# westlake-repl/IDvs.MoRec

Hardware: AMD Instinct MI355X
Metric: user-sequences/sec end-to-end train step, SASRec+BERT-base (higher is better)
Workload: dtype fp16

## Files before the change

### idvs/morec_amd/_lib.py

```python
from __future__ import annotations

import ctypes as C
import os

import torch

_HERE = os.path.dirname(os.path.abspath(__file__))
LIB_PATH = os.environ.get("MOREC_HIP_LIB") or os.path.join(_HERE, "libmorec_hip.so")

F32, BF16, F16 = 0, 1, 2
ACT_NONE, ACT_GELU, ACT_RELU = 0, 1, 2
DACT_MUL = 3


class MorecError(RuntimeError):
    pass


class GemmDesc(C.Structure):
    _fields_ = [("M", C.c_int), ("N", C.c_int), ("K", C.c_int), ("lda", C.c_int), ("ldb", C.c_int), ("ldc", C.c_int),
                ("in_dtype", C.c_int), ("out_dtype", C.c_int), ("act", C.c_int), ("dact", C.c_int),
                ("accumulate", C.c_int), ("split_k", C.c_int), ("alpha", C.c_float), ("aux_deriv", C.c_int)]


# ... 24 lines not shown
                ("pad0", C.c_int32), ("drop_seed", C.c_uint64), ("drop_seed_mixed", C.c_uint64), ("reserved", C.c_int32 * 2)]


class SwinAttnDesc(C.Structure):
    _fields_ = [("n_img", C.c_int), ("H", C.c_int), ("W", C.c_int), ("window", C.c_int), ("shift", C.c_int),
                ("heads", C.c_int), ("dh", C.c_int), ("scale", C.c_float), ("dtype", C.c_int)]


_P = C.c_void_p
_SIGS = {
    "morec_strerror": (C.c_char_p, [C.c_int]),
    "morec_version": (C.c_int, []),
    "morec_tuning_set": (C.c_int, [C.c_char_p, C.c_int]),
    "morec_det_scratch_reserve": (C.c_int, [C.c_size_t, C.c_void_p]),
    "morec_stream_wait_stream": (C.c_int, [_P, _P]),
    "morec_gemm_nt": (C.c_int, [C.POINTER(GemmDesc), _P, _P, _P, _P, _P, _P, _P]),
    "morec_gemm_nt_colsum": (C.c_int, [C.POINTER(GemmDesc), _P, _P, _P, _P, _P, _P, _P, _P, _P]),
    "morec_gemm_colsum_workspace_bytes": (C.c_size_t, [C.c_int, C.c_int]),
    "morec_gemm_plan": (C.c_int, [C.POINTER(GemmDesc), C.c_int, C.c_int, C.c_int, C.c_int, C.c_int, C.POINTER(GemmPlanInfo)]),
    "morec_gemm_tn": (C.c_int, [_P, _P, _P, C.c_int, C.c_int, C.c_int, C.c_int, C.c_int, C.c_int, C.c_int, C.c_int, C.c_int, _P, _P]),
    "morec_gemm_tn_workspace_bytes": (C.c_size_t, [C.c_int, C.c_int, C.c_int]),
    "morec_mlp_dact_recompute_supported": (C.c_int, [C.c_int, C.c_int, C.c_int, C.c_int]),
    "morec_mlp_dact_recompute_workspace_bytes": (C.c_size_t, [C.c_int]),
    "morec_mlp_dact_recompute": (C.c_int, [_P, _P, _P, _P, _P, _P, _P, _P, C.c_int, C.c_int, C.c_int, C.c_int, _P]),
    "morec_transpose": (C.c_int, [_P, _P, C.c_int, C.c_int, C.c_int, C.c_int, C.c_int, C.c_int, _P]),
    "morec_transpose_batch": (C.c_int, [_P, C.c_int, C.c_int, C.c_int, _P]),
    "morec_cast": (C.c_int, [_P, _P, C.c_size_t, C.c_int, C.c_int, _P]),
    "morec_split_bf16x3": (C.c_int, [_P, _P, C.c_int, C.c_int, C.c_int, C.c_int, C.c_int, _P]),
    "morec_act_bwd": (C.c_int, [_P, _P, _P, C.c_size_t, C.c_int, C.c_int, _P]),
    "morec_scaled_sum": (C.c_int, [_P, _P, _P, _P, C.c_size_t, C.c_float, C.c_int, _P]),
# ... 90 lines not shown
```

### idvs/morec_amd/csrc/attention.hip

```cpp
#include <stdio.h>
#include <stdlib.h>
#include "common.hpp"

namespace {
template <int TB>
struct Tile {
    static constexpr int TP = 8 * TB;
    static constexpr int PP = TP + 4;
};

struct AttnArgs {
    const void* qkv;
    const float* key_keep;
    void* ctx;
    void* dqkv;
    int n_seq, T, n_heads, dh;
    int causal;
    float scale, mask_value;
    DropRng drop;
    const int32_t* cu;
    int total_rows;
};

template <typename T, int DC, int TB>
// ... 670 lines not shown
    if (rc != MOREC_E_UNSUPPORTED) return rc;
    warn_valu_fallback(d);
    (void)block;
    if (d->T > Tile<8>::TP) return launch_long<true>(d, a, grid, s);
    return launch_valu<true>(d, a, grid, s);
}

extern "C" int morec_attn_bwd_dbias(const morec_attn_desc* d, const void* qkv, const float* key_keep, const void* dctx,
                                    void* dqkv, int rows, float* dbias, float* ws, size_t ws_bytes, void* stream) {
    int rc = check_desc(d);
    if (rc) return rc;
    if (!qkv || !key_keep || !dctx || !dqkv || !dbias || rows <= 0) return MOREC_E_ARG;
    const int H3 = 3 * d->n_heads * d->dh;
    hipStream_t s = reinterpret_cast<hipStream_t>(stream);
    if (ws && ws_bytes >= (size_t)d->n_seq * H3 * sizeof(float)) {
        rc = morec_attn_mfma_launch(d, qkv, key_keep, const_cast<void*>(dctx), dqkv, true, s, ws);
        if (rc == MOREC_OK) return colsum_f32_launch(ws, dbias, d->n_seq, H3, s);
        if (rc != MOREC_E_UNSUPPORTED) return rc;
    }
    rc = morec_attn_bwd(d, qkv, key_keep, dctx, dqkv, stream);
    if (rc) return rc;
    return morec_colsum(dqkv, dbias, rows, H3, H3, d->dtype, stream);
}
```

### idvs/morec_amd/csrc/capi.hip

```cpp
#include <atomic>
#include <mutex>
#include <stdlib.h>
#include "common.hpp"

extern "C" const char* morec_strerror(int code) {
    switch (code) {
        case MOREC_OK: return "ok";
        case MOREC_E_ARG: return "MOREC_E_ARG: null pointer or non-positive size";
        case MOREC_E_ALIGN: return "MOREC_E_ALIGN: pointer/pitch not 16-byte aligned or size not a vector multiple";
        case MOREC_E_UNSUPPORTED: return "MOREC_E_UNSUPPORTED: shape outside kernel limits";
        case MOREC_E_DTYPE: return "MOREC_E_DTYPE: unsupported dtype combination";
        case MOREC_E_COMM: return "MOREC_E_COMM: an RCCL call failed (morec_comm_last_error)";
        default: break;
    }
    if (code > 0) return hipGetErrorString(static_cast<hipError_t>(code));
    return "unknown morec error";
}

extern "C" int morec_version(void) { return 105; }

static const uint64_t* g_drop_seed_src = nullptr;
const uint64_t* morec_drop_seed_src() { return g_drop_seed_src; }
extern "C" int morec_dropout_seed_source(const void* dev_u64) {
    if (reinterpret_cast<uintptr_t>(dev_u64) & 7u) return MOREC_E_ALIGN;
    g_drop_seed_src = reinterpret_cast<const uint64_t*>(dev_u64);
    return MOREC_OK;
}

static float* det_scratch_impl(hipStream_t s, size_t n, bool may_grow) {
    struct Slot { hipStream_t s; int dev; float* p; size_t n; unsigned long long used; };
    static Slot slots[16];
    static int n_slots = 0;
    static unsigned long long tick = 0;
    static std::mutex mu;
    std::lock_guard<std::mutex> lock(mu);
    int dev = 0;
    (void)hipGetDevice(&dev);
    hipStreamCaptureStatus cap = hipStreamCaptureStatusNone;
    if (hipStreamIsCapturing(s, &cap) != hipSuccess) { (void)hipGetLastError(); cap = hipStreamCaptureStatusNone; }
    const bool capturing = cap != hipStreamCaptureStatusNone;
    Slot* sl = nullptr;
    for (int i = 0; i < n_slots; ++i)
        if (slots[i].s == s && slots[i].dev == dev) sl = &slots[i];
    if (!sl) {
        if (capturing || !may_grow) return nullptr;
        if (n_slots < 16) {
            sl = &slots[n_slots++];
        } else {
            for (int i = 0; i < n_slots; ++i)
                if (slots[i].dev == dev && (!sl || slots[i].used < sl->used)) sl = &slots[i];
            if (!sl) return nullptr;
            (void)hipDeviceSynchronize();
            if (sl->p) (void)hipFree(sl->p);
        }
        *sl = Slot{s, dev, nullptr, 0, 0};
    }
    sl->used = ++tick;
    if (sl->n < n) {
        if (capturing || !may_grow) return nullptr;
        if (sl->p) {
            (void)hipStreamSynchronize(s);
            (void)hipFree(sl->p);
            sl->p = nullptr; sl->n = 0;
        }
        size_t want = n + n / 4;
        if (want < ((size_t)1 << 20)) want = (size_t)1 << 20;
        if (hipMalloc(reinterpret_cast<void**>(&sl->p), want * sizeof(float)) != hipSuccess) { (void)hipGetLastError(); sl->p = nullptr; return nullptr; }
        sl->n = want;
    }
    return sl->p;
}
float* morec_det_scratch(hipStream_t s, size_t n) { return det_scratch_impl(s, n, true); }
extern "C" int morec_det_scratch_reserve(size_t n_floats, void* stream) {
    return det_scratch_impl(reinterpret_cast<hipStream_t>(stream), n_floats, true) ? MOREC_OK : (int)hipErrorOutOfMemory;
}

__global__ __launch_bounds__(256) void det_fold_add_kernel(const float* __restrict__ part, float* __restrict__ dst, int n_parts, size_t n, size_t stride) {
    __shared__ float red[16][17];
    const int c = threadIdx.x & 15, g = threadIdx.x >> 4;
    const size_t j = blockIdx.x * (size_t)16 + c;
    float a0 = 0.f, a1 = 0.f, a2 = 0.f, a3 = 0.f;
    if (j < n) {
        int p = g;
        for (; p + 48 < n_parts; p += 64) {
            a0 += part[(size_t)p * stride + j];
            a1 += part[(size_t)(p + 16) * stride + j];
            a2 += part[(size_t)(p + 32) * stride + j];
            a3 += part[(size_t)(p + 48) * stride + j];
        }
        for (; p < n_parts; p += 16) a0 += part[(size_t)p * stride + j];
    }
    red[g][c] = (a0 + a1) + (a2 + a3);
    __syncthreads();
    if (g == 0 && j < n) {
        float t = 0.f;
#pragma unroll
        for (int k = 0; k < 16; ++k) t += red[k][c];
        dst[j] += t;
    }
}
int morec_det_fold_add(const float* part, float* dst, int n_parts, size_t n, size_t stride, hipStream_t s) {
    if (n == 0 || n_parts <= 0) return MOREC_OK;
    hipLaunchKernelGGL(det_fold_add_kernel, dim3((unsigned)((n + 15) / 16)), dim3(256), 0, s, part, dst, n_parts, n, stride);
    MOREC_CHECK_LAUNCH();
    return MOREC_OK;
}

extern "C" int morec_stream_wait_stream(void* waiting, void* signal) {
    static hipEvent_t ring[256];
    static std::atomic<unsigned> next{0};
    static const hipError_t made = [] {
        for (auto& e : ring) {
            const hipError_t rc = hipEventCreateWithFlags(&e, hipEventDisableTiming);
            if (rc != hipSuccess) return rc;
        }
        return hipSuccess;
    }();
    if (made != hipSuccess) return (int)made;
    hipEvent_t e = ring[next.fetch_add(1u, std::memory_order_relaxed) & 255u];
// ... 61 lines not shown
```

### idvs/morec_amd/csrc/common.hpp

```cpp
#pragma once
#include <hip/hip_runtime.h>
#include <stdint.h>
#include <math.h>
#include <type_traits>
#include "morec_hip.h"
#include "tuning.hpp"

#define MOREC_WAVE 64

struct bf16 {
    unsigned short v;
};

typedef __attribute__((ext_vector_type(8))) __bf16 bf16x8_t;
typedef __attribute__((ext_vector_type(4))) float f32x4_t;

__device__ __forceinline__ float bf2f(bf16 x) { return __uint_as_float(((uint32_t)x.v) << 16); }
__device__ __forceinline__ float bfbits2f(uint32_t lo16) { return __uint_as_float(lo16 << 16); }
typedef __attribute__((ext_vector_type(2))) float f32x2_t;
typedef __attribute__((ext_vector_type(2))) __bf16 bf16x2_t;
typedef __attribute__((ext_vector_type(4))) __bf16 bf16x4_t;
__device__ __forceinline__ unsigned short f2bf_bits(float f) { return __builtin_bit_cast(unsigned short, (__bf16)f); }
__device__ __forceinline__ uint32_t pack_bf16x2(float lo, float hi) {
    const f32x2_t v = {lo, hi};
// ... 336 lines not shown
        case MOREC_F16: f((f16*)nullptr); return true;
        default: return false;
    }
}
#define MOREC_TAG_T(tag) typename std::remove_pointer<decltype(tag)>::type
#define MOREC_CHECK_LAUNCH()                        \
    do {                                            \
        hipError_t e__ = hipGetLastError();         \
        if (e__ != hipSuccess) return (int)e__;     \
    } while (0)

bool morec_deterministic();
void morec_set_deterministic(int on);
float* morec_det_scratch(hipStream_t s, size_t n);
int morec_det_fold_add(const float* part, float* dst, int n_parts, size_t n, size_t stride, hipStream_t s);

__device__ __forceinline__ int xcd_remap(int bid, int nwg) {
    const int q = nwg >> 3, r = nwg & 7, xcd = bid & 7, idx = bid >> 3;
    const int base = (xcd < r) ? xcd * (q + 1) : r * (q + 1) + (xcd - r) * q;
    return base + idx;
}
```

### idvs/morec_amd/csrc/gemm.hip

```cpp
#include "gemm_nt_generic.hpp"


extern "C" int morec_gemm_nt(const morec_gemm_desc* d, const void* A, const void* B, void* C, const float* bias,
                             void* aux_out, const void* dact_in, void* stream) {
    return morec_gemm_nt_colsum(d, A, B, C, bias, aux_out, dact_in, nullptr, nullptr, stream);
}

extern "C" size_t morec_gemm_colsum_workspace_bytes(int M, int N) {
    return (size_t)((M + 31) / 32) * (size_t)N * sizeof(float);
}

static int check_gemm_desc(const morec_gemm_desc* d, bool aligned, bool dact_in, bool aux_out, bool colsum) {
    if (colsum) {
        if (d->dact == MOREC_ACT_NONE || d->accumulate != 0 || d->split_k > 1) return MOREC_E_UNSUPPORTED;
        const int os_ = elt_size(d->out_dtype);
        if ((d->N * os_) % 16 || (d->ldc * os_) % 16) return MOREC_E_UNSUPPORTED;
    }
    if (d->M <= 0 || d->N <= 0 || d->K <= 0) return MOREC_E_ARG;
    const int es = elt_size(d->in_dtype), os = elt_size(d->out_dtype);
    if (!aligned) return MOREC_E_ALIGN;
    if ((d->lda * es) % 16 || (d->ldb * es) % 16 || (d->K * es) % 16) return MOREC_E_ALIGN;
    if (d->N % 4 || (d->ldc * os) % (4 * os) || d->ldc % 4) return MOREC_E_ALIGN;
    if (d->split_k > 1 && d->accumulate != 2) return MOREC_E_ARG;
    if (d->accumulate == 2 && d->out_dtype != MOREC_F32) return MOREC_E_DTYPE;
// ... 8 lines not shown
    return (d->N * os) % 16 == 0 && (d->ldc * os) % 16 == 0;
}

extern "C" int morec_gemm_nt_colsum(const morec_gemm_desc* d, const void* A, const void* B, void* C, const float* bias,
                                    void* aux_out, const void* dact_in, float* colsum_out, float* workspace, void* stream) {
    if (!d || !A || !B || !C) return MOREC_E_ARG;
    if (colsum_out && !workspace) return MOREC_E_ARG;
    const bool aligned = aligned16(A) && aligned16(B) && aligned16(C) && (!bias || aligned16(bias));
    const int rc = check_gemm_desc(d, aligned, dact_in, aux_out, colsum_out);
    if (rc) return rc;
    GemmArgs a{};
    a.A = A; a.B = B; a.C = C; a.bias = bias; a.aux_out = aux_out; a.dact_in = dact_in;
    a.M = d->M; a.N = d->N; a.K = d->K; a.lda = d->lda; a.ldb = d->ldb; a.ldc = d->ldc;
    a.act = d->act; a.dact = d->dact; a.accumulate = d->accumulate; a.alpha = d->alpha;
    a.aux_deriv = d->aux_deriv;
    a.colsum = colsum_out ? workspace : nullptr;
    a.colsum_dst = colsum_out;
    a.vec_store = rows_16_byte_addressable(d) && (!aux_out || aligned16(aux_out));
    const GemmOperands o{bias != nullptr, aux_out != nullptr, dact_in != nullptr, colsum_out != nullptr, a.vec_store != 0, aligned16(bias)};
    const GemmPlan p = gemm_plan(*d, o, tuning(), gemm8p_cu_count());
    a.wave_epilogue = p.wave_epilogue;
    hipStream_t s = reinterpret_cast<hipStream_t>(stream);
    switch (p.family) {
        case GEMM_SKINNY: return gemm_skinny_launch(p, a, s);
        case GEMM_SKINNY_WIDE: return gemm_skinny_wide_launch(p, a, s);
        case GEMM_TWO_W: return gemm2w_launch(p, a, s);
        case GEMM_EIGHT_P: return gemm8p_launch(p, a, s);
        case GEMM_SMALL: return gemm_small_launch(p, a, s);
        case GEMM_GENERIC:
            if (p.in_dtype == MOREC_F16) return gemm_nt_f16_launch(p, a, s);
// ... 204 lines not shown
            float t = 0.f;
#pragma unroll
            for (int r = 0; r < 16; ++r) t += part[r][threadIdx.x];
            if (det) out[(size_t)blockIdx.y * N + c] = t;
            else atomicAdd(out + c, t);
        }
    }
}

int colsum_f32_launch(const float* in, float* out, int rows, int N, hipStream_t s) {
    const int cb = (N + 63) / 64;
    int rpb = (int)(((long)rows * cb / 512 + 15) & ~15L);
    rpb = rpb < 16 ? 16 : rpb > 512 ? 512 : rpb;
    if ((long)rows * N <= (1L << 20) && rows <= 512) rpb = 512;
    dim3 grid(cb, (rows + rpb - 1) / rpb);
    if (grid.y > 1 && morec_deterministic()) {
        float* part = morec_det_scratch(s, (size_t)grid.y * N);
        if (!part) return (int)hipErrorOutOfMemory;
        hipLaunchKernelGGL((colsum_kernel<float>), grid, dim3(256), 0, s, in, part, rows, N, N, rpb, 1);
        MOREC_CHECK_LAUNCH();
        return morec_det_fold_add(part, out, (int)grid.y, (size_t)N, (size_t)N, s);
    }
    hipLaunchKernelGGL((colsum_kernel<float>), grid, dim3(256), 0, s, in, out, rows, N, N, rpb);
    MOREC_CHECK_LAUNCH();
    return MOREC_OK;
}

extern "C" int morec_colsum(const void* in, float* out, int M, int N, int ld, int dtype, void* stream) {
    if (!in || !out || M <= 0 || N <= 0) return MOREC_E_ARG;
    if (N % 4 || ld % 4) return MOREC_E_ALIGN;
    const int rpb = 512;
    dim3 grid((N + 63) / 64, (M + rpb - 1) / rpb);
    hipStream_t s = reinterpret_cast<hipStream_t>(stream);
    float* part = nullptr;
    if (grid.y > 1 && morec_deterministic()) {
        part = morec_det_scratch(s, (size_t)grid.y * N);
        if (!part) return (int)hipErrorOutOfMemory;
    }
    if (!by_dtype(dtype, [&](auto* t) {
            using T = MOREC_TAG_T(t);
            hipLaunchKernelGGL((colsum_kernel<T>), grid, dim3(256), 0, s, (const T*)in, part ? part : out, M, N, ld, rpb, part ? 1 : 0);
        }))
        return MOREC_E_DTYPE;
    MOREC_CHECK_LAUNCH();
    if (part) return morec_det_fold_add(part, out, (int)grid.y, (size_t)N, (size_t)N, s);
    return MOREC_OK;
}

template <typename T>
__global__ void act_bwd_kernel(const T* __restrict__ dy, const T* __restrict__ pre, T* __restrict__ out, size_t n4,
// ... 66 lines not shown
```

### idvs/morec_amd/csrc/gemm_skinny_wide.hip

```cpp
#include "gemm_core.hpp"
#include "gemm_args.hpp"

namespace {
typedef __attribute__((ext_vector_type(4))) unsigned int u32x4_t;
constexpr int TR = 32;
constexpr int THREADS = 512;
constexpr int NW = 8;

struct WArgs {
    const bf16* A;
    const bf16* B;
    bf16* C;
    const float* bias;
    const bf16* A2;
    const bf16* B2;
    float* colsum_ws;
    int M, N, K, lda, ldb, ldc, lda2, ldb2, tiles;
};

template <int N>
__device__ __forceinline__ void vm_wait() {
    asm volatile("s_waitcnt vmcnt(%0)" ::"n"(N) : "memory");
}
__device__ __forceinline__ void bar_lds() {
// ... 251 lines not shown

extern "C" int morec_mlp_dact_recompute(const void* dY, const void* W2t, const void* X, const void* W1, const float* b1, void* dU,
                                        float* colsum_out, float* workspace, int M, int N, int K, int dtype, void* stream) {
    if (!dY || !W2t || !X || !W1 || !dU || M <= 0 || N <= 0 || K <= 0) return MOREC_E_ARG;
    if (colsum_out && !workspace) return MOREC_E_ARG;
    if (!is_h16(dtype)) return MOREC_E_DTYPE;
    if (!dual_class_exists(M, N, K, dtype)) return MOREC_E_UNSUPPORTED;
    if (b1 && (reinterpret_cast<uintptr_t>(b1) & 15u)) return MOREC_E_ALIGN;
    if (!aligned16(dY) || !aligned16(W2t) || !aligned16(X) || !aligned16(W1) || !aligned16(dU)) return MOREC_E_ALIGN;
    hipStream_t s = reinterpret_cast<hipStream_t>(stream);
    WArgs k{};
    k.A = reinterpret_cast<const bf16*>(dY); k.B = reinterpret_cast<const bf16*>(W2t); k.C = reinterpret_cast<bf16*>(dU);
    k.A2 = reinterpret_cast<const bf16*>(X); k.B2 = reinterpret_cast<const bf16*>(W1);
    k.bias = b1;
    k.M = M; k.N = N; k.K = K; k.lda = K; k.ldb = K; k.ldc = N; k.lda2 = K; k.ldb2 = K; k.tiles = (M + TR - 1) / TR;
    k.colsum_ws = colsum_out ? workspace : nullptr;
    return dtype == MOREC_F16 ? dispatch_wide<f16, 1, true>(k, colsum_out, s) : dispatch_wide<bf16, 1, true>(k, colsum_out, s);
}
```

### idvs/morec_amd/csrc/swin.hip

```cpp
#include <algorithm>
#include "common.hpp"

namespace {
constexpr int DH = 32;

struct SwinAttnArgs {
    const void* qkv;
    const float* bias_t;
    void* ctx;
    const void* dctx;
    void* dqkv;
    float* dbias_t;
    float* dbias_part;
    int n_img, H, W, shift, heads;
    float scale;
    int n_win_total, wpb;
};

template <int WS>
__device__ __forceinline__ void token_geom(const SwinAttnArgs& a, int img, int wr, int wc, int t, int& row, int& reg) {
    const int wy = t / WS, wx = t - wy * WS;
    const int ys = wr * WS + wy, xs = wc * WS + wx;
    int y = ys + a.shift, x = xs + a.shift;
    if (y >= a.H) y -= a.H;
// ... 468 lines not shown
    hipStream_t s = reinterpret_cast<hipStream_t>(stream);
    rc = morec_swin_attn_mfma_launch(d, qkv, bias_t, const_cast<void*>(ctx), dctx, dqkv, dbias_t, true, s);
    if (rc != MOREC_E_UNSUPPORTED) return rc;
    dim3 grid(gx, d->heads), block(64);
    const int NT2 = d->window * d->window * d->window * d->window;
    if (dbias_t && morec_deterministic()) {
        a.dbias_part = morec_det_scratch(s, (size_t)d->heads * gx * NT2);
        if (!a.dbias_part) return (int)hipErrorOutOfMemory;
    }
    if (d->dtype == MOREC_F32) hipLaunchKernelGGL((swin_attn_bwd_kernel<float, 7>), grid, block, 0, s, a);
    else if (d->dtype == MOREC_F16) hipLaunchKernelGGL((swin_attn_bwd_kernel<f16, 7>), grid, block, 0, s, a);
    else hipLaunchKernelGGL((swin_attn_bwd_kernel<bf16, 7>), grid, block, 0, s, a);
    MOREC_CHECK_LAUNCH();
    if (a.dbias_part)
        for (int h = 0; h < d->heads; ++h) {
            rc = morec_det_fold_add(a.dbias_part + (size_t)h * gx * NT2, dbias_t + (size_t)h * NT2, gx, (size_t)NT2, (size_t)NT2, s);
            if (rc) return rc;
        }
    return MOREC_OK;
}

extern "C" int morec_swin_bias_expand(const float* table, float* bias_t, int window, int heads, void* stream) {
    if (!table || !bias_t || window <= 0 || heads <= 0) return MOREC_E_ARG;
    const int n = heads * window * window * window * window;
    hipLaunchKernelGGL(swin_bias_expand_kernel, dim3((n + 255) / 256), dim3(256), 0, reinterpret_cast<hipStream_t>(stream),
                       table, bias_t, window, heads);
    MOREC_CHECK_LAUNCH();
    return MOREC_OK;
}

extern "C" int morec_swin_bias_reduce(const float* dbias_t, float* dtable, int window, int heads, void* stream) {
// ... 122 lines not shown
    MOREC_CHECK_LAUNCH();
    return MOREC_OK;
}

extern "C" int morec_swin_attn_bwd_dbias(const morec_swin_attn_desc* d, const void* qkv, const float* bias_t, const void* ctx,
                                         const void* dctx, void* dqkv, float* dbias_t, float* dbqkv, float* ws, size_t ws_bytes,
                                         void* stream) {
    int rc = check_attn(d);
    if (rc) return rc;
    if (!qkv || !bias_t || !ctx || !dctx || !dqkv || !dbqkv) return MOREC_E_ARG;
    const int C3 = 3 * d->heads * d->dh;
    const long rows = (long)d->n_img * d->H * d->W;
    hipStream_t s = reinterpret_cast<hipStream_t>(stream);
    if (ws) {
        int need = 0;
        rc = morec_swin_attn_mfma_launch(d, qkv, bias_t, const_cast<void*>(ctx), dctx, dqkv, dbias_t, true, s, ws,
                                         (long)(ws_bytes / (C3 * sizeof(float))), &need);
        if (rc == MOREC_OK) return colsum_f32_launch(ws, dbqkv, need, C3, s);
        if (rc != MOREC_E_UNSUPPORTED) return rc;
    }
    rc = morec_swin_attn_bwd(d, qkv, bias_t, ctx, dctx, dqkv, dbias_t, stream);
    if (rc) return rc;
    return morec_colsum(dqkv, dbqkv, (int)rows, C3, C3, d->dtype, stream);
}
```

### idvs/morec_amd/csrc/swin_attn_mfma.hip

```cpp
#include <algorithm>
#include <stdlib.h>
#include <type_traits>
#include "common.hpp"

namespace {
constexpr int DH = 32;
constexpr int WS = 7, NT = WS * WS;
constexpr int TROW = 64;
constexpr int TILE = 64 * TROW;
constexpr int PROW = 136;
constexpr int PTILE = 64 * PROW;
constexpr int BP = 68;
#ifndef SWIN_BWD_NTI
#define SWIN_BWD_NTI 2
#endif
typedef __attribute__((ext_vector_type(4))) short s16x4_t;
typedef __attribute__((ext_vector_type(8))) short s16x8_t;
typedef __attribute__((address_space(3))) s16x4_t* lds_s16x4_ptr;

struct SwinMArgs {
    const bf16* qkv;
    const float* bias_t;
    bf16* ctx;
    const bf16* dctx;
// ... 590 lines not shown
            hipLaunchKernelGGL(swin_attn_fwd_mfma_kernel<T>, grid, block, 0, s, a);
            return;
        }
        static const bool attr_set = [&] {
            (void)hipFuncSetAttribute(reinterpret_cast<const void*>(&swin_attn_bwd_mfma_kernel<T, false>), hipFuncAttributeMaxDynamicSharedMemorySize, (int)lds);
            (void)hipFuncSetAttribute(reinterpret_cast<const void*>(&swin_attn_bwd_mfma_kernel<T, true>), hipFuncAttributeMaxDynamicSharedMemorySize, (int)lds);
            return true;
        }();
        (void)attr_set;
        if (wide) hipLaunchKernelGGL((swin_attn_bwd_mfma_kernel<T, true>), grid, block, lds, s, a);
        else hipLaunchKernelGGL((swin_attn_bwd_mfma_kernel<T, false>), grid, block, lds, s, a);
    });
    MOREC_CHECK_LAUNCH();
    if (a.dbias_part)
        for (int h = 0; h < d->heads; ++h) {
            const int rc = morec_det_fold_add(a.dbias_part + (size_t)h * a.gx * (NT * NT), dbias_t + (size_t)h * (NT * NT), a.gx, (size_t)(NT * NT), (size_t)(NT * NT), s);
            if (rc) return rc;
        }
    return MOREC_OK;
}
```

### idvs/morec_amd/csrc/tuning.hip

```cpp
#include <stdlib.h>
#include <string.h>
#include "common.hpp"

namespace {
enum Handling {
    RAW,
    FLAG,
    TMR,
    RESERVE,
    TAIL_BIAS,
    AT_LEAST_1,
    NOT_CHAR_0,
    IS_CHAR_1,
    EPI,
};
struct Row {
    const char* key;
    const char* env;
    int Tuning::*field;
    int def;
    Handling how;
};
const Row ROWS[] = {
    {"gemm8p", "MOREC_GEMM8P", &Tuning::gemm8p, 0, RAW},
    {"gemm2w", "MOREC_GEMM2W", &Tuning::gemm2w, 0, RAW},
    {"gemm_small", "MOREC_GEMM_SMALL", &Tuning::gemm_small, 0, RAW},
    {"gemm_skinny", "MOREC_GEMM_SKINNY", &Tuning::gemm_skinny, 0, RAW},
    {"ce8p", "MOREC_CE8P", &Tuning::ce8p, 0, RAW},
    {"gemm8p_tmr", "MOREC_GEMM8P_TMR", &Tuning::gemm8p_tmr, 1, TMR},
    {"gemm8p_ngroup", "MOREC_GEMM8P_NGROUP", &Tuning::gemm8p_ngroup, -1, RAW},
    {"gemm8p_reserve_cus", "MOREC_GEMM8P_RESERVE_CUS", &Tuning::gemm8p_reserve_cus, 0, RESERVE},
    {"gemm8p_tail_split", "MOREC_GEMM8P_TAIL_SPLIT", &Tuning::gemm8p_tail_split, 0, FLAG},
    {"gemm8p_tail_bias", nullptr, &Tuning::gemm8p_tail_bias, 2, TAIL_BIAS},
    {"gemm8p_debug", "MOREC_GEMM8P_DEBUG", &Tuning::gemm8p_debug, 0, RAW},
    {"gemm8p_stamps_lo", nullptr, &Tuning::gemm8p_stamps_lo, 0, RAW},
    {"gemm8p_stamps_hi", nullptr, &Tuning::gemm8p_stamps_hi, 0, RAW},
    {"deterministic", "MOREC_DETERMINISTIC", &Tuning::deterministic, 0, FLAG},
    {nullptr, "MOREC_GEMM_TILE", &Tuning::gemm_tile, 0, RAW},
    {nullptr, "MOREC_GEMM_EPI", &Tuning::gemm_epi, 2, EPI},
    {nullptr, "MOREC_GEMM2W_STAGGER", &Tuning::gemm2w_stagger, 0, RAW},
    {nullptr, "MOREC_TN8P_SKIP", &Tuning::tn8p_skip, 1, FLAG},
    {nullptr, "MOREC_ATTN_MFMA64", &Tuning::attn_mfma64, 1, NOT_CHAR_0},
    {nullptr, "MOREC_ATTN_F32_MFMA", &Tuning::attn_f32_mfma, 1, NOT_CHAR_0},
    {nullptr, "MOREC_SWIN_WPW_MIN", &Tuning::swin_wpw_min, 8, AT_LEAST_1},
    {nullptr, "MOREC_SWIN_BWD_WIDE", &Tuning::swin_bwd_wide, 1, RAW},
    {nullptr, "MOREC_QUIET", &Tuning::quiet, 0, IS_CHAR_1},
};

int handled(Handling how, int v) {
    switch (how) {
        case FLAG: return v != 0;
        case TMR: return (v == 0 || v == 1 || v == 224 || v == 192) ? v : 1;
// ... 55 lines not shown
```

### idvs/morec_amd/csrc/tuning.hpp

```cpp
#pragma once

struct Tuning {
    int gemm8p, gemm2w, gemm_small, gemm_skinny, ce8p;
    int gemm8p_tmr;
    int gemm8p_ngroup;
    int gemm8p_reserve_cus;
    int gemm8p_tail_split, gemm8p_tail_bias;
    int gemm8p_debug;
    int gemm8p_stamps_lo, gemm8p_stamps_hi;
    int deterministic;
    int gemm_tile;
    int gemm_epi;
    int gemm2w_stagger;
    int tn8p_skip;
    int attn_mfma64;
    int attn_f32_mfma;
    int swin_wpw_min;
    int swin_bwd_wide;
    int quiet;

    unsigned long long gemm8p_stamps() const {
        return ((unsigned long long)(unsigned)gemm8p_stamps_hi << 32) | (unsigned)gemm8p_stamps_lo;
    }
};

// ... 5 lines not shown
```

### idvs/morec_amd/ops.py

```python
from __future__ import annotations

import ctypes as C
import os

import torch

from . import _lib
from ._lib import ACT_GELU, ACT_NONE, ACT_RELU, BF16, F16, F32, AttnDesc, CeDesc, GemmDesc, SwinAttnDesc, check

FLT_MIN_MASK = -3.4028234663852886e38


DETERMINISTIC = _lib.env_flag("MOREC_DETERMINISTIC")


def set_deterministic(on: bool = True):
    global DETERMINISTIC
    check(_lib.lib().morec_tuning_set(b"deterministic", int(bool(on))), "morec_tuning_set(deterministic)")
    DETERMINISTIC = bool(on)


def code(dt: torch.dtype) -> int:
    if dt == torch.float32:
        return F32
# ... 7 lines not shown
def _p(t):
    return None if t is None else t.data_ptr()


_raw_stream = None if os.environ.get("MOREC_STREAM_OBJ") == "1" else getattr(torch._C, "_cuda_getCurrentRawStream", None)


def _stream():
    if _raw_stream is not None:
        return _raw_stream(torch.cuda.current_device())
    return torch.cuda.current_stream().cuda_stream


def stream_wait_stream(waiting, signal=None):
    check(_lib.lib().morec_stream_wait_stream(waiting, _stream() if signal is None else signal), "morec_stream_wait_stream")


def _dev(t):
    if not t.is_cuda:
        raise _lib.MorecError("libmorec_hip needs device tensors (no CPU fallback)")
    if not t.is_contiguous():
        raise _lib.MorecError("tensor must be contiguous")
    return t


def is16(dt: torch.dtype) -> bool:
    return dt in (torch.bfloat16, torch.float16)


def pad8(n: int) -> int:
# ... 661 lines not shown
```

### idvs/morec_amd/train_step.py

```python
from __future__ import annotations

import os
import re
from collections import OrderedDict

import torch
import torch.distributed as dist

from . import engine, ops, swin_engine
from .functional import pool_exchange, reduce_scatter_dE


def _round8(n: int) -> int:
    return (n + 7) & ~7


class ParamArena:

    def __init__(self, named_params, device, shadow):
        shadow = torch.bfloat16 if shadow is True else (shadow or None)
        self.offsets = OrderedDict()
        off = 0
        for name, p in named_params:
            self.offsets[name] = (off, p.numel(), tuple(p.shape))
# ... 117 lines not shown
                                    lr=fine_tune_lr, wd=fine_tune_l2_weight))
        self.groups.append(dict(arena=ParamArena([(n, named[n]) for n in g1], self.device, use_shadow), lr=lr, wd=l2_weight))
        self.frozen = {n: p.data for n, p in named.items() if n not in set(g0) | set(g1)}
        self._build_views()
        self._build_transposed_shadows()
        self.world = dist.get_world_size() if (dist.is_available() and dist.is_initialized()) else 1
        self.rank = dist.get_rank() if self.world > 1 else 0
        if force_collectives and not (dist.is_available() and dist.is_initialized()):
            raise ValueError("force_collectives needs an initialised process group")
        self.collectives = self.world > 1 or bool(force_collectives)
        self.overlap_reduce = os.environ.get("MOREC_OVERLAP_REDUCE", "1") != "0"
        rccl_ring = (self.world > 1 and self.overlap_reduce and self.device.type == "cuda" and dist.is_initialized() and dist.get_backend() != "gloo")
        env_r = os.environ.get("MOREC_GEMM8P_RESERVE_CUS")
        self.reserve_cus = (int(env_r) if env_r is not None else 16) if rccl_ring else 0
        self._reserved = False
        comm = comm if comm is not None else os.environ.get("MOREC_COMM", "")
        self.comm = self.comm_grad = self._grad_stream = None
        if comm == "rccl" and self.collectives and self.device.type == "cuda":
            from .comm import MorecComm
            self.comm, self.comm_grad = MorecComm(), MorecComm()
            self._grad_stream = torch.cuda.Stream(device=self.device)
        self.log_pop = torch.log(model.pop_prob_list).to(self.device)
        self.sp = None
        self._param_ready = {}
        if graph is None:
            graph = os.environ.get("MOREC_GRAPH", "0") == "1"
        self.graph = bool(graph) and self.device.type == "cuda" and not self.collectives and not self.dedup_items
        if self.dtype == torch.float16 or loss_scale is not None or self.graph or os.environ.get("MOREC_STEP_PARAMS", "0") == "1":
            init = float(loss_scale) if loss_scale is not None else (65536.0 if self.dtype == torch.float16 else 1.0)
            self.sp = ops.StepParams(self.device, init_scale=init, step=0, growth_interval=growth_interval,
# ... 192 lines not shown
        if dedup:
            E_u = E
            E = ops.gather_rows(ops.cast(E_u, torch.float32) if E_u.dtype != torch.float32 else E_u, inv32, self.dtype)
        B = log_mask.shape[0]
        x_in = E.view(B, S + 1, D)[:, :-1, :].contiguous()
        prep_s = engine.sasrec_prepare(p, m.args.transformer_block, self.dtype, engine.UE, self.sh)
        P, saved_s = engine.sasrec_forward(p, prep_s, x_in, log_mask, m.args.num_attention_heads, True, engine.UE, d_user, res32=self.res32)
        if side is not None:
            torch.cuda.current_stream(self.device).wait_stream(side)
        Epool = E
        if self.collectives and self.pool:
            Epool, ci, n_valid = pool_exchange(E, ci, n_valid, self.world, self.rank, self.comm)
            gscale = self._gscale(n_valid)
        loss_sum, saved_c = engine.ce_forward(ci, P, Epool, dE_fp32=(self.collectives and self.pool))
        self._reserve(True)
        dP, dEpool = engine.ce_backward(ci, P, Epool, saved_c, gscale, 1.0)
        dE = reduce_scatter_dE(dEpool, self.world, self.rank, self.dtype, self.comm) if (self.collectives and self.pool) else dEpool
        dx = engine.sasrec_backward(p, prep_s, saved_s, dP, grads, engine.UE)
        dE.view(B, S + 1, D)[:, :-1, :].add_(dx.view(B, S, D))
        if dedup:
            dE_u = torch.zeros((E_u.shape[0], D), device=dE.device, dtype=torch.float32)
            ops.scatter_add_rows_(dE.contiguous(), inv32, dE_u, -1)
            dE = dE_u if self.dtype == torch.float32 else ops.cast(dE_u, self.dtype)
        if self.vision:
            swin_engine.swin_backward(p, prep_b, saved_b, dE, grads, swin_engine.IN, on_ready=self._on_ready)
        elif m.use_modal:
            d_pass = dE if len(passes) == 1 else ops.scaled_sum([dE.contiguous()], 1.0 / len(passes))
            for ai, (_, saved_a) in enumerate(passes):
                engine.bert_backward(p, prep_b, saved_a, d_pass, grads, engine.TE, on_ready=self._on_ready if ai == len(passes) - 1 else None)
        else:
            ops.scatter_add_rows_(dE, idx32, grads["id_embedding.weight"], 0)
        engine.WgradStream.join(self.device)
        ops.x3_cache_clear()
        return loss_sum[0] / n_valid

    def _begin_step(self):
        if self._decide_first and not self._decided:
            self.sp.decide_(self.betas[0], self.betas[1])
            self._decided = True

    def _gscale(self, n_valid):
        if self.sp is None:
            return (1.0 / n_valid).reshape(1)
        return (self.sp.loss_scale_dev / n_valid).reshape(1)

    def _reserve(self, on: bool):
        if self.reserve_cus <= 0 or on == self._reserved:
# ... 26 lines not shown
        if self.comm_grad is not None:
            self._grad_stream.wait_stream(torch.cuda.current_stream())
            with torch.cuda.stream(self._grad_stream):
                self.comm_grad.all_reduce_sum_(t)
                if self.trace is not None:
                    ev = torch.cuda.Event(enable_timing=True)
                    ev.record(self._grad_stream)
                    self.trace.append(("done", gi, lo, hi, ev))
            self._pending.append(None)
        elif dist.get_backend() == "gloo":
            self._all_reduce(t)
        else:
            self._pending.append(dist.all_reduce(t, async_op=True))
        self._reduced.append((gi, lo, hi))

    def _on_ready(self, key):
        if not self.collectives:
            self._early_adamw(key)
            return
        if not self.overlap_reduce:
            return
        side = engine.WgradStream.get(self.device) if self.device in engine.WgradStream._dirty else None
        if side is not None:
            side.wait_stream(torch.cuda.current_stream(self.device))
            with torch.cuda.stream(side):
                self._issue_ready(key)
            return
        self._issue_ready(key)

    def _early_adamw(self, key):
        if not self._fused_update or (self.sp is not None and not self._decide_first):
# ... 322 lines not shown
```

### include/morec_hip.h

```cpp
#ifndef MOREC_HIP_H
#define MOREC_HIP_H

#include <stddef.h>
#include <stdint.h>

#ifdef __cplusplus
extern "C" {
#endif

#define MOREC_F32 0
#define MOREC_BF16 1
#define MOREC_F16 2

#define MOREC_OK 0
#define MOREC_E_ARG (-1)
#define MOREC_E_ALIGN (-2)
#define MOREC_E_UNSUPPORTED (-3)
#define MOREC_E_DTYPE (-4)
#define MOREC_E_COMM (-5)

#define MOREC_ACT_NONE 0
#define MOREC_ACT_GELU 1
#define MOREC_ACT_RELU 2
#define MOREC_DACT_MUL 3

const char* morec_strerror(int code);
int morec_version(void);
int morec_tuning_set(const char* key, int value);
int morec_det_scratch_reserve(size_t n_floats, void* stream);

typedef struct {
    int M, N, K;
    int lda, ldb, ldc;
    int in_dtype;
    int out_dtype;
    int act;
    int dact;
    int accumulate;
    int split_k;
    float alpha;
    int aux_deriv;
} morec_gemm_desc;

int morec_gemm_nt(const morec_gemm_desc* d, const void* A, const void* B, void* C, const float* bias,
// ... 207 lines not shown
```

Before: 3599.

## Defer deterministic gradient fold reductions and batch them into one side-stream launch

In deterministic mode, the per-GEMM, attention and colsum fold-add reductions issued during backward are queued instead of launched right away, each with its own bump-allocated scratch region. Queued jobs are flushed as batched multi-job kernels, up to 64 non-overlapping jobs per launch, on the weight-grad side stream at on_ready points and at the end of backward. The aim is to cut many small kernel launches and take reduction work off the critical stream. The cost is extra scratch memory, a host-side mutex, extra work in defer_end, and new ordering dependencies between the side stream and the main stream.

```diff
diff --git a/idvs/morec_amd/_lib.py b/idvs/morec_amd/_lib.py
--- a/idvs/morec_amd/_lib.py
+++ b/idvs/morec_amd/_lib.py
@@ -62,6 +62,11 @@
     "morec_tuning_set": (C.c_int, [C.c_char_p, C.c_int]),
     "morec_det_scratch_reserve": (C.c_int, [C.c_size_t, C.c_void_p]),
     "morec_stream_wait_stream": (C.c_int, [_P, _P]),
+    "morec_fold_defer_begin": (C.c_int, [_P]),
+    "morec_fold_defer_active": (C.c_int, []),
+    "morec_fold_flush": (C.c_int, [_P]),
+    "morec_fold_defer_end": (C.c_int, []),
+    "morec_fold_stats": (C.c_int, [_P]),
     "morec_gemm_nt": (C.c_int, [C.POINTER(GemmDesc), _P, _P, _P, _P, _P, _P, _P]),
     "morec_gemm_nt_colsum": (C.c_int, [C.POINTER(GemmDesc), _P, _P, _P, _P, _P, _P, _P, _P, _P]),
     "morec_gemm_colsum_workspace_bytes": (C.c_size_t, [C.c_int, C.c_int]),
diff --git a/idvs/morec_amd/csrc/attention.hip b/idvs/morec_amd/csrc/attention.hip
--- a/idvs/morec_amd/csrc/attention.hip
+++ b/idvs/morec_amd/csrc/attention.hip
@@ -708,6 +708,8 @@
     const int H3 = 3 * d->n_heads * d->dh;
     hipStream_t s = reinterpret_cast<hipStream_t>(stream);
     if (ws && ws_bytes >= (size_t)d->n_seq * H3 * sizeof(float)) {
+        ws = morec_fold_workspace(ws, (size_t)d->n_seq * H3, s);
+        if (!ws) return (int)hipErrorOutOfMemory;
         rc = morec_attn_mfma_launch(d, qkv, key_keep, const_cast<void*>(dctx), dqkv, true, s, ws);
         if (rc == MOREC_OK) return colsum_f32_launch(ws, dbias, d->n_seq, H3, s);
         if (rc != MOREC_E_UNSUPPORTED) return rc;
diff --git a/idvs/morec_amd/csrc/capi.hip b/idvs/morec_amd/csrc/capi.hip
--- a/idvs/morec_amd/csrc/capi.hip
+++ b/idvs/morec_amd/csrc/capi.hip
@@ -1,6 +1,7 @@
 #include <atomic>
 #include <mutex>
 #include <stdlib.h>
+#include <vector>
 #include "common.hpp"
 
 extern "C" const char* morec_strerror(int code) {
@@ -27,7 +28,8 @@
     return MOREC_OK;
 }
 
-static float* det_scratch_impl(hipStream_t s, size_t n, bool may_grow) {
+float* morec_det_scratch(hipStream_t s, size_t n) {
+    if (morec_fold_deferring(s)) return morec_fold_scratch(s, n);
     struct Slot { hipStream_t s; int dev; float* p; size_t n; unsigned long long used; };
     static Slot slots[16];
     static int n_slots = 0;
@@ -43,7 +45,7 @@
     for (int i = 0; i < n_slots; ++i)
         if (slots[i].s == s && slots[i].dev == dev) sl = &slots[i];
     if (!sl) {
-        if (capturing || !may_grow) return nullptr;
+        if (capturing) return nullptr;
         if (n_slots < 16) {
             sl = &slots[n_slots++];
         } else {
@@ -57,7 +59,7 @@
     }
     sl->used = ++tick;
     if (sl->n < n) {
-        if (capturing || !may_grow) return nullptr;
+        if (capturing) return nullptr;
         if (sl->p) {
             (void)hipStreamSynchronize(s);
             (void)hipFree(sl->p);
@@ -70,9 +72,8 @@
     }
     return sl->p;
 }
-float* morec_det_scratch(hipStream_t s, size_t n) { return det_scratch_impl(s, n, true); }
 extern "C" int morec_det_scratch_reserve(size_t n_floats, void* stream) {
-    return det_scratch_impl(reinterpret_cast<hipStream_t>(stream), n_floats, true) ? MOREC_OK : (int)hipErrorOutOfMemory;
+    return morec_det_scratch(reinterpret_cast<hipStream_t>(stream), n_floats) ? MOREC_OK : (int)hipErrorOutOfMemory;
 }
 
 __global__ __launch_bounds__(256) void det_fold_add_kernel(const float* __restrict__ part, float* __restrict__ dst, int n_parts, size_t n, size_t stride) {
@@ -101,8 +102,207 @@
 }
 int morec_det_fold_add(const float* part, float* dst, int n_parts, size_t n, size_t stride, hipStream_t s) {
     if (n == 0 || n_parts <= 0) return MOREC_OK;
+    if (morec_fold_defer(part, dst, n, n_parts, stride, 0, s)) return MOREC_OK;
+    return morec_det_fold_add_now(part, dst, n_parts, n, stride, s);
+}
+int morec_det_fold_add_now(const float* part, float* dst, int n_parts, size_t n, size_t stride, hipStream_t s) {
+    if (n == 0 || n_parts <= 0) return MOREC_OK;
     hipLaunchKernelGGL(det_fold_add_kernel, dim3((unsigned)((n + 15) / 16)), dim3(256), 0, s, part, dst, n_parts, n, stride);
     MOREC_CHECK_LAUNCH();
+    return MOREC_OK;
+}
+
+namespace {
+constexpr int FOLD_MAX_JOBS = 64;
+struct FoldJob {
+    const float* src;
+    float* dst;
+    unsigned n;
+    unsigned cnt;
+    unsigned stride;
+    unsigned rpb;
+    unsigned blk0;
+    unsigned pad_;
+};
+struct FoldBatch {
+    int n_jobs, pad_;
+    FoldJob job[FOLD_MAX_JOBS];
+};
+struct FoldChunk { float* p; size_t n; };
+struct FoldState {
+    std::mutex mu;
+    bool open = false;
+    hipStream_t producer = nullptr;
+    std::vector<FoldJob> queue;
+    std::vector<FoldChunk> chunks;
+    size_t used = 0;
+    unsigned long long n_alloc = 0, n_jobs = 0, n_launch = 0;
+};
+FoldState g_fold;
+constexpr size_t FOLD_ALIGN = 64;
+constexpr size_t FOLD_CHUNK_MIN = (size_t)16 << 20;
+}
+
+__global__ __launch_bounds__(256) void fold_batch_kernel(const FoldBatch b) {
+    int ji = 0;
+    while (ji + 1 < b.n_jobs && blockIdx.x >= b.job[ji + 1].blk0) ++ji;
+    const float* __restrict__ src = b.job[ji].src;
+    float* __restrict__ dst = b.job[ji].dst;
+    const unsigned n = b.job[ji].n, rpb = b.job[ji].rpb;
+    const int cnt = (int)b.job[ji].cnt;
+    const size_t stride = b.job[ji].stride;
+    const int lane = threadIdx.x & 63, c = lane & 3, g = lane >> 2;
+    const size_t j = ((size_t)(blockIdx.x - b.job[ji].blk0) * 4 + (threadIdx.x >> 6)) * 4 + c;
+    const bool live = j < n;
+    float a0 = 0.f, a1 = 0.f, a2 = 0.f, a3 = 0.f;
+    if (rpb == 0) {
+        if (live) {
+            int p = g;
+            for (; p + 48 < cnt; p += 64) {
+                a0 += src[(size_t)p * stride + j];
+                a1 += src[(size_t)(p + 16) * stride + j];
+                a2 += src[(size_t)(p + 32) * stride + j];
+                a3 += src[(size_t)(p + 48) * stride + j];
+            }
+            for (; p < cnt; p += 16) a0 += src[(size_t)p * stride + j];
+        }
+    } else {
+        const int nb = (cnt + (int)rpb - 1) / (int)rpb;
+        for (int blk = 0; blk < nb; ++blk) {
+            const int r0 = blk * (int)rpb, r1 = min(cnt, r0 + (int)rpb);
+            float s = 0.f;
+            if (live) {
+#pragma unroll 4
+                for (int r = r0 + g; r < r1; r += 16) s += src[(size_t)r * stride + j];
+            }
+            float t = 0.f;
+#pragma unroll
+            for (int k = 0; k < 16; ++k) t += __shfl(s, k * 4 + c);
+            const int gi = blk & 15;
+            const int ch = ((blk & ~63) + gi + 48 < nb) ? (blk >> 4) & 3 : 0;
+            if (g == gi) {
+                if (ch == 0) a0 += t;
+                else if (ch == 1) a1 += t;
+                else if (ch == 2) a2 += t;
+                else a3 += t;
+            }
+        }
+    }
+    const float v = (a0 + a1) + (a2 + a3);
+    float t = 0.f;
+#pragma unroll
+    for (int k = 0; k < 16; ++k) t += __shfl(v, k * 4 + c);
+    if (g == 0 && live) dst[j] += t;
+}
+
+bool morec_fold_deferring(hipStream_t s) {
+    std::lock_guard<std::mutex> lock(g_fold.mu);
+    return g_fold.open && g_fold.producer == s;
+}
+
+float* morec_fold_scratch(hipStream_t s, size_t n) {
+    (void)s;
+    std::lock_guard<std::mutex> lock(g_fold.mu);
+    n = (n + FOLD_ALIGN - 1) & ~(FOLD_ALIGN - 1);
+    if (g_fold.chunks.empty() || g_fold.used + n > g_fold.chunks.back().n) {
+        FoldChunk ck{nullptr, n > FOLD_CHUNK_MIN ? n : FOLD_CHUNK_MIN};
+        if (hipMalloc(reinterpret_cast<void**>(&ck.p), ck.n * sizeof(float)) != hipSuccess) { (void)hipGetLastError(); return nullptr; }
+        ++g_fold.n_alloc;
+        g_fold.chunks.push_back(ck);
+        g_fold.used = 0;
+    }
+    float* p = g_fold.chunks.back().p + g_fold.used;
+    g_fold.used += n;
+    return p;
+}
+
+bool morec_fold_defer(const float* src, float* dst, size_t n, int cnt, size_t stride, int rpb, hipStream_t s) {
+    std::lock_guard<std::mutex> lock(g_fold.mu);
+    if (!g_fold.open || g_fold.producer != s) return false;
+    if (n == 0 || cnt <= 0) return true;
+    if (n > 0xffffffffu || stride > 0xffffffffu) return false;
+    g_fold.queue.push_back(FoldJob{src, dst, (unsigned)n, (unsigned)cnt, (unsigned)stride, (unsigned)rpb, 0u, 0u});
+    ++g_fold.n_jobs;
+    return true;
+}
+
+extern "C" int morec_fold_defer_begin(void* stream) {
+    hipStream_t s = reinterpret_cast<hipStream_t>(stream);
+    if (!tuning().fold_defer || !morec_deterministic()) return MOREC_OK;
+    hipStreamCaptureStatus cap = hipStreamCaptureStatusNone;
+    if (hipStreamIsCapturing(s, &cap) != hipSuccess) { (void)hipGetLastError(); cap = hipStreamCaptureStatusNone; }
+    if (cap != hipStreamCaptureStatusNone) return MOREC_OK;
+    std::lock_guard<std::mutex> lock(g_fold.mu);
+    if (g_fold.open) return g_fold.producer == s ? MOREC_OK : MOREC_E_UNSUPPORTED;
+    g_fold.open = true;
+    g_fold.producer = s;
+    return MOREC_OK;
+}
+
+extern "C" int morec_fold_defer_active(void) {
+    std::lock_guard<std::mutex> lock(g_fold.mu);
+    return g_fold.open ? 1 : 0;
+}
+
+extern "C" int morec_fold_flush(void* stream) {
+    hipStream_t s = reinterpret_cast<hipStream_t>(stream);
+    std::lock_guard<std::mutex> lock(g_fold.mu);
+    const std::vector<FoldJob>& q = g_fold.queue;
+    size_t i = 0;
+    while (i < q.size()) {
+        FoldBatch batch;
+        batch.n_jobs = 0;
+        batch.pad_ = 0;
+        unsigned blocks = 0;
+        for (; i < q.size() && batch.n_jobs < FOLD_MAX_JOBS; ++i) {
+            bool overlap = false;
+            for (int k = 0; k < batch.n_jobs && !overlap; ++k)
+                overlap = q[i].dst < batch.job[k].dst + batch.job[k].n && batch.job[k].dst < q[i].dst + q[i].n;
+            if (overlap) break;
+            FoldJob& j = batch.job[batch.n_jobs++];
+            j = q[i];
+            j.blk0 = blocks;
+            blocks += (j.n + 15) / 16;
+        }
+        hipLaunchKernelGGL(fold_batch_kernel, dim3(blocks), dim3(256), 0, s, batch);
+        ++g_fold.n_launch;
+        const hipError_t e = hipGetLastError();
+        if (e != hipSuccess) { g_fold.queue.clear(); return (int)e; }
+    }
+    g_fold.queue.clear();
+    return MOREC_OK;
+}
+
+extern "C" int morec_fold_defer_end(void) {
+    std::lock_guard<std::mutex> lock(g_fold.mu);
+    if (!g_fold.open) return MOREC_OK;
+    g_fold.open = false;
+    g_fold.producer = nullptr;
+    g_fold.queue.clear();
+    g_fold.used = 0;
+    if (g_fold.chunks.size() > 1) {
+        size_t total = 0;
+        for (const FoldChunk& ck : g_fold.chunks) total += ck.n;
+        (void)hipDeviceSynchronize();
+        for (const FoldChunk& ck : g_fold.chunks) (void)hipFree(ck.p);
+        g_fold.chunks.clear();
+        FoldChunk ck{nullptr, total + total / 4};
+        if (hipMalloc(reinterpret_cast<void**>(&ck.p), ck.n * sizeof(float)) != hipSuccess) { (void)hipGetLastError(); return (int)hipErrorOutOfMemory; }
+        ++g_fold.n_alloc;
+        g_fold.chunks.push_back(ck);
+    }
+    return MOREC_OK;
+}
+
+extern "C" int morec_fold_stats(unsigned long long* out4) {
+    if (!out4) return MOREC_E_ARG;
+    std::lock_guard<std::mutex> lock(g_fold.mu);
+    size_t cap = 0;
+    for (const FoldChunk& ck : g_fold.chunks) cap += ck.n;
+    out4[0] = g_fold.n_alloc;
+    out4[1] = (unsigned long long)cap * sizeof(float);
+    out4[2] = g_fold.n_jobs;
+    out4[3] = g_fold.n_launch;
     return MOREC_OK;
 }
 
diff --git a/idvs/morec_amd/csrc/common.hpp b/idvs/morec_amd/csrc/common.hpp
--- a/idvs/morec_amd/csrc/common.hpp
+++ b/idvs/morec_amd/csrc/common.hpp
@@ -374,6 +374,13 @@
 void morec_set_deterministic(int on);
 float* morec_det_scratch(hipStream_t s, size_t n);
 int morec_det_fold_add(const float* part, float* dst, int n_parts, size_t n, size_t stride, hipStream_t s);
+int morec_det_fold_add_now(const float* part, float* dst, int n_parts, size_t n, size_t stride, hipStream_t s);
+bool morec_fold_deferring(hipStream_t s);
+float* morec_fold_scratch(hipStream_t s, size_t n);
+bool morec_fold_defer(const float* src, float* dst, size_t n, int cnt, size_t stride, int rpb, hipStream_t s);
+static inline float* morec_fold_workspace(float* ws, size_t n_floats, hipStream_t s) {
+    return (ws && morec_deterministic() && morec_fold_deferring(s)) ? morec_fold_scratch(s, n_floats) : ws;
+}
 
 __device__ __forceinline__ int xcd_remap(int bid, int nwg) {
     const int q = nwg >> 3, r = nwg & 7, xcd = bid & 7, idx = bid >> 3;
diff --git a/idvs/morec_amd/csrc/gemm.hip b/idvs/morec_amd/csrc/gemm.hip
--- a/idvs/morec_amd/csrc/gemm.hip
+++ b/idvs/morec_amd/csrc/gemm.hip
@@ -7,7 +7,7 @@
 }
 
 extern "C" size_t morec_gemm_colsum_workspace_bytes(int M, int N) {
-    return (size_t)((M + 31) / 32) * (size_t)N * sizeof(float);
+    return ((size_t)((M + 255) / 256) * 8 + 8) * (size_t)N * sizeof(float);
 }
 
 static int check_gemm_desc(const morec_gemm_desc* d, bool aligned, bool dact_in, bool aux_out, bool colsum) {
@@ -46,6 +46,10 @@
     a.M = d->M; a.N = d->N; a.K = d->K; a.lda = d->lda; a.ldb = d->ldb; a.ldc = d->ldc;
     a.act = d->act; a.dact = d->dact; a.accumulate = d->accumulate; a.alpha = d->alpha;
     a.aux_deriv = d->aux_deriv;
+    if (colsum_out) {
+        workspace = morec_fold_workspace(workspace, morec_gemm_colsum_workspace_bytes(d->M, d->N) / sizeof(float), reinterpret_cast<hipStream_t>(stream));
+        if (!workspace) return (int)hipErrorOutOfMemory;
+    }
     a.colsum = colsum_out ? workspace : nullptr;
     a.colsum_dst = colsum_out;
     a.vec_store = rows_16_byte_addressable(d) && (!aux_out || aligned16(aux_out));
@@ -280,6 +284,7 @@
     rpb = rpb < 16 ? 16 : rpb > 512 ? 512 : rpb;
     if ((long)rows * N <= (1L << 20) && rows <= 512) rpb = 512;
     dim3 grid(cb, (rows + rpb - 1) / rpb);
+    if (morec_deterministic() && morec_fold_defer(in, out, (size_t)N, rows, (size_t)N, rpb, s)) return MOREC_OK;
     if (grid.y > 1 && morec_deterministic()) {
         float* part = morec_det_scratch(s, (size_t)grid.y * N);
         if (!part) return (int)hipErrorOutOfMemory;
@@ -299,7 +304,7 @@
     dim3 grid((N + 63) / 64, (M + rpb - 1) / rpb);
     hipStream_t s = reinterpret_cast<hipStream_t>(stream);
     float* part = nullptr;
-    if (grid.y > 1 && morec_deterministic()) {
+    if (morec_deterministic() && (grid.y > 1 || morec_fold_deferring(s))) {
         part = morec_det_scratch(s, (size_t)grid.y * N);
         if (!part) return (int)hipErrorOutOfMemory;
     }
diff --git a/idvs/morec_amd/csrc/gemm_skinny_wide.hip b/idvs/morec_amd/csrc/gemm_skinny_wide.hip
--- a/idvs/morec_amd/csrc/gemm_skinny_wide.hip
+++ b/idvs/morec_amd/csrc/gemm_skinny_wide.hip
@@ -289,6 +289,10 @@
     k.A2 = reinterpret_cast<const bf16*>(X); k.B2 = reinterpret_cast<const bf16*>(W1);
     k.bias = b1;
     k.M = M; k.N = N; k.K = K; k.lda = K; k.ldb = K; k.ldc = N; k.lda2 = K; k.ldb2 = K; k.tiles = (M + TR - 1) / TR;
+    if (colsum_out) {
+        workspace = morec_fold_workspace(workspace, morec_mlp_dact_recompute_workspace_bytes(N) / sizeof(float), s);
+        if (!workspace) return (int)hipErrorOutOfMemory;
+    }
     k.colsum_ws = colsum_out ? workspace : nullptr;
     return dtype == MOREC_F16 ? dispatch_wide<f16, 1, true>(k, colsum_out, s) : dispatch_wide<bf16, 1, true>(k, colsum_out, s);
 }
diff --git a/idvs/morec_amd/csrc/swin.hip b/idvs/morec_amd/csrc/swin.hip
--- a/idvs/morec_amd/csrc/swin.hip
+++ b/idvs/morec_amd/csrc/swin.hip
@@ -506,7 +506,7 @@
     MOREC_CHECK_LAUNCH();
     if (a.dbias_part)
         for (int h = 0; h < d->heads; ++h) {
-            rc = morec_det_fold_add(a.dbias_part + (size_t)h * gx * NT2, dbias_t + (size_t)h * NT2, gx, (size_t)NT2, (size_t)NT2, s);
+            rc = morec_det_fold_add_now(a.dbias_part + (size_t)h * gx * NT2, dbias_t + (size_t)h * NT2, gx, (size_t)NT2, (size_t)NT2, s);
             if (rc) return rc;
         }
     return MOREC_OK;
@@ -659,6 +659,8 @@
     hipStream_t s = reinterpret_cast<hipStream_t>(stream);
     if (ws) {
         int need = 0;
+        ws = morec_fold_workspace(ws, ws_bytes / sizeof(float), s);
+        if (!ws) return (int)hipErrorOutOfMemory;
         rc = morec_swin_attn_mfma_launch(d, qkv, bias_t, const_cast<void*>(ctx), dctx, dqkv, dbias_t, true, s, ws,
                                          (long)(ws_bytes / (C3 * sizeof(float))), &need);
         if (rc == MOREC_OK) return colsum_f32_launch(ws, dbqkv, need, C3, s);
diff --git a/idvs/morec_amd/csrc/swin_attn_mfma.hip b/idvs/morec_amd/csrc/swin_attn_mfma.hip
--- a/idvs/morec_amd/csrc/swin_attn_mfma.hip
+++ b/idvs/morec_amd/csrc/swin_attn_mfma.hip
@@ -628,7 +628,7 @@
     MOREC_CHECK_LAUNCH();
     if (a.dbias_part)
         for (int h = 0; h < d->heads; ++h) {
-            const int rc = morec_det_fold_add(a.dbias_part + (size_t)h * a.gx * (NT * NT), dbias_t + (size_t)h * (NT * NT), a.gx, (size_t)(NT * NT), (size_t)(NT * NT), s);
+            const int rc = morec_det_fold_add_now(a.dbias_part + (size_t)h * a.gx * (NT * NT), dbias_t + (size_t)h * (NT * NT), a.gx, (size_t)(NT * NT), (size_t)(NT * NT), s);
             if (rc) return rc;
         }
     return MOREC_OK;
diff --git a/idvs/morec_amd/csrc/tuning.hip b/idvs/morec_amd/csrc/tuning.hip
--- a/idvs/morec_amd/csrc/tuning.hip
+++ b/idvs/morec_amd/csrc/tuning.hip
@@ -36,6 +36,7 @@
     {"gemm8p_stamps_lo", nullptr, &Tuning::gemm8p_stamps_lo, 0, RAW},
     {"gemm8p_stamps_hi", nullptr, &Tuning::gemm8p_stamps_hi, 0, RAW},
     {"deterministic", "MOREC_DETERMINISTIC", &Tuning::deterministic, 0, FLAG},
+    {"fold_defer", "MOREC_FOLD_DEFER", &Tuning::fold_defer, 1, FLAG},
     {nullptr, "MOREC_GEMM_TILE", &Tuning::gemm_tile, 0, RAW},
     {nullptr, "MOREC_GEMM_EPI", &Tuning::gemm_epi, 2, EPI},
     {nullptr, "MOREC_GEMM2W_STAGGER", &Tuning::gemm2w_stagger, 0, RAW},
diff --git a/idvs/morec_amd/csrc/tuning.hpp b/idvs/morec_amd/csrc/tuning.hpp
--- a/idvs/morec_amd/csrc/tuning.hpp
+++ b/idvs/morec_amd/csrc/tuning.hpp
@@ -9,6 +9,7 @@
     int gemm8p_debug;
     int gemm8p_stamps_lo, gemm8p_stamps_hi;
     int deterministic;
+    int fold_defer;
     int gemm_tile;
     int gemm_epi;
     int gemm2w_stagger;
diff --git a/idvs/morec_amd/ops.py b/idvs/morec_amd/ops.py
--- a/idvs/morec_amd/ops.py
+++ b/idvs/morec_amd/ops.py
@@ -45,6 +45,26 @@
 
 def stream_wait_stream(waiting, signal=None):
     check(_lib.lib().morec_stream_wait_stream(waiting, _stream() if signal is None else signal), "morec_stream_wait_stream")
+
+
+def fold_defer_begin() -> bool:
+    h = _lib.lib()
+    check(h.morec_fold_defer_begin(_stream()), "morec_fold_defer_begin")
+    return bool(h.morec_fold_defer_active())
+
+
+def fold_flush(stream=None):
+    check(_lib.lib().morec_fold_flush(_stream() if stream is None else stream), "morec_fold_flush")
+
+
+def fold_defer_end():
+    check(_lib.lib().morec_fold_defer_end(), "morec_fold_defer_end")
+
+
+def fold_stats() -> dict:
+    out = (C.c_ulonglong * 4)()
+    check(_lib.lib().morec_fold_stats(out), "morec_fold_stats")
+    return {"allocations": out[0], "scratch_bytes": out[1], "jobs": out[2], "launches": out[3]}
 
 
 def _dev(t):
diff --git a/idvs/morec_amd/train_step.py b/idvs/morec_amd/train_step.py
--- a/idvs/morec_amd/train_step.py
+++ b/idvs/morec_amd/train_step.py
@@ -155,6 +155,7 @@
         env_r = os.environ.get("MOREC_GEMM8P_RESERVE_CUS")
         self.reserve_cus = (int(env_r) if env_r is not None else 16) if rccl_ring else 0
         self._reserved = False
+        self._fold_open = False
         comm = comm if comm is not None else os.environ.get("MOREC_COMM", "")
         self.comm = self.comm_grad = self._grad_stream = None
         if comm == "rccl" and self.collectives and self.device.type == "cuda":
@@ -377,23 +378,30 @@
             gscale = self._gscale(n_valid)
         loss_sum, saved_c = engine.ce_forward(ci, P, Epool, dE_fp32=(self.collectives and self.pool))
         self._reserve(True)
-        dP, dEpool = engine.ce_backward(ci, P, Epool, saved_c, gscale, 1.0)
-        dE = reduce_scatter_dE(dEpool, self.world, self.rank, self.dtype, self.comm) if (self.collectives and self.pool) else dEpool
-        dx = engine.sasrec_backward(p, prep_s, saved_s, dP, grads, engine.UE)
-        dE.view(B, S + 1, D)[:, :-1, :].add_(dx.view(B, S, D))
-        if dedup:
-            dE_u = torch.zeros((E_u.shape[0], D), device=dE.device, dtype=torch.float32)
-            ops.scatter_add_rows_(dE.contiguous(), inv32, dE_u, -1)
-            dE = dE_u if self.dtype == torch.float32 else ops.cast(dE_u, self.dtype)
-        if self.vision:
-            swin_engine.swin_backward(p, prep_b, saved_b, dE, grads, swin_engine.IN, on_ready=self._on_ready)
-        elif m.use_modal:
-            d_pass = dE if len(passes) == 1 else ops.scaled_sum([dE.contiguous()], 1.0 / len(passes))
-            for ai, (_, saved_a) in enumerate(passes):
-                engine.bert_backward(p, prep_b, saved_a, d_pass, grads, engine.TE, on_ready=self._on_ready if ai == len(passes) - 1 else None)
-        else:
-            ops.scatter_add_rows_(dE, idx32, grads["id_embedding.weight"], 0)
-        engine.WgradStream.join(self.device)
+        self._fold_open = ops.fold_defer_begin()
+        try:
+            dP, dEpool = engine.ce_backward(ci, P, Epool, saved_c, gscale, 1.0)
+            dE = reduce_scatter_dE(dEpool, self.world, self.rank, self.dtype, self.comm) if (self.collectives and self.pool) else dEpool
+            dx = engine.sasrec_backward(p, prep_s, saved_s, dP, grads, engine.UE)
+            dE.view(B, S + 1, D)[:, :-1, :].add_(dx.view(B, S, D))
+            if dedup:
+                dE_u = torch.zeros((E_u.shape[0], D), device=dE.device, dtype=torch.float32)
+                ops.scatter_add_rows_(dE.contiguous(), inv32, dE_u, -1)
+                dE = dE_u if self.dtype == torch.float32 else ops.cast(dE_u, self.dtype)
+            if self.vision:
+                swin_engine.swin_backward(p, prep_b, saved_b, dE, grads, swin_engine.IN, on_ready=self._on_ready)
+            elif m.use_modal:
+                d_pass = dE if len(passes) == 1 else ops.scaled_sum([dE.contiguous()], 1.0 / len(passes))
+                for ai, (_, saved_a) in enumerate(passes):
+                    engine.bert_backward(p, prep_b, saved_a, d_pass, grads, engine.TE, on_ready=self._on_ready if ai == len(passes) - 1 else None)
+            else:
+                ops.scatter_add_rows_(dE, idx32, grads["id_embedding.weight"], 0)
+            self._fold_flush()
+            engine.WgradStream.join(self.device)
+        finally:
+            if self._fold_open:
+                self._fold_open = False
+                ops.fold_defer_end()
         ops.x3_cache_clear()
         return loss_sum[0] / n_valid
 
@@ -450,7 +458,20 @@
             self._pending.append(dist.all_reduce(t, async_op=True))
         self._reduced.append((gi, lo, hi))
 
+    def _fold_flush(self):
+        if not self._fold_open:
+            return
+        side = engine.WgradStream.get(self.device)
+        if side is None:
+            ops.fold_flush()
+            return
+        sh = side.cuda_stream
+        ops.stream_wait_stream(sh)
+        ops.fold_flush(sh)
+        engine.WgradStream._dirty.add(self.device)
+
     def _on_ready(self, key):
+        self._fold_flush()
         if not self.collectives:
             self._early_adamw(key)
             return
diff --git a/include/morec_hip.h b/include/morec_hip.h
--- a/include/morec_hip.h
+++ b/include/morec_hip.h
@@ -28,6 +28,11 @@
 int morec_version(void);
 int morec_tuning_set(const char* key, int value);
 int morec_det_scratch_reserve(size_t n_floats, void* stream);
+int morec_fold_defer_begin(void* stream);
+int morec_fold_defer_active(void);
+int morec_fold_flush(void* run_on);
+int morec_fold_defer_end(void);
+int morec_fold_stats(unsigned long long* out4);
 
 typedef struct {
     int M, N, K;
```

Result: faster. 3638 (median of 6 runs) (+1.1%).
